# HarryShomer/LPFormer

Hardware: AMD Instinct MI355X
Metric: candidate link-pairs scored/sec (whole node) (higher is better)
Workload: dtype f32

## Files before the change

### lpformer_amd/csrc/tail_chain.hip

```cpp
#include <type_traits>

#include "lpf_common.h"

namespace {

typedef float f32x4 __attribute__((ext_vector_type(4)));

#ifndef LPF_TC_GROUPS
#define LPF_TC_GROUPS 4
#endif
constexpr int TC_GROUPS = LPF_TC_GROUPS;
constexpr int TC_WAVES = 2 * TC_GROUPS;
constexpr int TC_THREADS = 64 * TC_WAVES;

struct TailArgs {
    int64_t M;
    const float *x; int64_t ldx; int KA;
    const float *addend; int64_t ldadd;
    const float *wA, *lnA_g, *lnA_b; int NA;
    const float *tail; int64_t ldtail;
    const float *wB, *bB, *lnB_g, *lnB_b; int NB;
    const float *re; int64_t ldre;
    const float *wC, *bC; int NC;
    const float *wdot, *bdot;
    float *logit, *prob;
    const float *part;
    const float *bnd;
    int64_t units_cap;
    const int32_t *type_ptr;
    const float *att_bias;
    const int64_t *sel_ctl;
    int n_counts;
    const float *rows; int64_t ldrows;
    const int32_t *perm;
    const int64_t *n_full;
    const float *bC_empty;
    const float *row_empty;
    const float *X; int64_t ldX;
    const int64_t *batch; int64_t batch_ld, n_rows;
    const float *wE, *bE, *lnE_g, *lnE_b;
};

constexpr int tc_per_thread(int ntp) { return (ntp * 64 + TC_THREADS - 1) / TC_THREADS; }
constexpr int tc_stage_stride(int ntp) { return (ntp * 64 + 511) / 512 * 512; }

typedef short bf16x4_bits __attribute__((ext_vector_type(4)));
template <int P, int NTP, typename T>
__device__ __forceinline__ void tc_load(T (&r)[P], const float *packed, int stage, int tid) {
    const T *src = reinterpret_cast<const T *>(packed) + (int64_t)stage * tc_stage_stride(NTP);
#pragma unroll
    for (int e = 0; e < P; ++e) {
        const int i = e * TC_THREADS + tid;
#ifdef TC_NOWLOAD
        r[e] = T{};
        (void)src; (void)i;
#else
        r[e] = src[i < tc_stage_stride(NTP) ? i : 0];
#endif
    }
}
template <int P, typename T>
__device__ __forceinline__ void tc_store(const T (&r)[P], T *slab, int tid) {
#pragma unroll
    for (int e = 0; e < P; ++e) slab[e * TC_THREADS + tid] = r[e];
}

template <int TPW>
__device__ __forceinline__ void tc_mfma(f32x4 (&acc)[TPW], const f32x4 *lw, const f32x4 bv, bool last = true) {
    f32x4 a[TPW];
#pragma unroll
    for (int c = 0; c < TPW; ++c) a[c] = lw[c * 64];
#pragma unroll
    for (int u = 0; u < 4; ++u) {
#pragma unroll
        for (int c = 0; c < TPW - 1; ++c) acc[c] = __builtin_amdgcn_mfma_f32_16x16x4f32(a[c][u], bv[u], acc[c], 0, 0, 0);
        if (last) acc[TPW - 1] = __builtin_amdgcn_mfma_f32_16x16x4f32(a[TPW - 1][u], bv[u], acc[TPW - 1], 0, 0, 0);
    }
}
template <int TPW>
__device__ __forceinline__ void tc_mfma(f32x4 (&acc)[TPW], const uint2 *lw, const f32x4 bv, bool last = true) {
    bf16x4_bits b;
#pragma unroll
    for (int u = 0; u < 4; ++u) b[u] = (short)lpf_f32_to_bf16(bv[u]);
#pragma unroll
    for (int c = 0; c < TPW; ++c) {
        if (c == TPW - 1 && !last) break;
        const uint2 w = lw[c * 64];
        const bf16x4_bits a = {(short)(w.x & 0xffffu), (short)(w.x >> 16), (short)(w.y & 0xffffu), (short)(w.y >> 16)};
        acc[c] = __builtin_amdgcn_mfma_f32_16x16x16bf16_1k(a, b, acc[c], 0, 0, 0);
    }
}

template <int TPW>
__device__ __forceinline__ void tc_layernorm(f32x4 (&acc)[TPW], int fbase, int n, const float *g, const float *b, int half,
                                             int q, float *my_x, const float *peer_x, bool relu) {
    float s1 = 0.f;
#pragma unroll
    for (int c = 0; c < TPW; ++c) s1 += acc[c][0] + acc[c][1] + acc[c][2] + acc[c][3];
    s1 = lpf_quad_sum(s1);
    __syncthreads();
    if (q == 0) *my_x = s1;
    __syncthreads();
    const float mean = (half == 0 ? s1 + *peer_x : *peer_x + s1) / (float)n;
    float s2 = 0.f;
#pragma unroll
    for (int c = 0; c < TPW; ++c)
#pragma unroll
        for (int r = 0; r < 4; ++r) {
            const float d = (fbase + 16 * c + r < n) ? acc[c][r] - mean : 0.f;
            s2 += d * d;
        }
    s2 = lpf_quad_sum(s2);
    __syncthreads();
    if (q == 0) *my_x = s2;
    __syncthreads();
    const float rstd = 1.0f / sqrtf((half == 0 ? s2 + *peer_x : *peer_x + s2) / (float)n + 1e-5f);
#pragma unroll
    for (int c = 0; c < TPW; ++c) {
        const f32x4 gg = *reinterpret_cast<const f32x4 *>(g + fbase + 16 * c);
        const f32x4 bb = *reinterpret_cast<const f32x4 *>(b + fbase + 16 * c);
        acc[c] = (acc[c] - mean) * rstd * gg + bb;
        if (relu) {
#pragma unroll
            for (int r = 0; r < 4; ++r) acc[c][r] = fmaxf(acc[c][r], 0.f);
        }
    }
}

#ifdef TC_STAMPS
__device__ uint64_t *tc_stamp_buf = nullptr;
#define TC_STAMP(k) do { if (lane == 0) st_t[k] = wall_clock64(); } while (0)
#define TC_STAMPS_OUT(kind) do { if (lane == 0 && tc_stamp_buf) { uint64_t *o__ = tc_stamp_buf + ((int64_t)blockIdx.x * TC_WAVES + wave) * 16; \
        for (int k__ = 0; k__ < 8; ++k__) o__[k__] = st_t[k__]; o__[15] = (kind); } } while (0)
#else
#define TC_STAMP(k) do { } while (0)
#define TC_STAMPS_OUT(kind) do { } while (0)
#endif

template <int NTA, int NTB, int NTC>
struct TcShape {
    static constexpr int NTPA = (NTA + 1) & ~1, NTPB = (NTB + 1) & ~1, NTPC = (NTC + 1) & ~1;
    static constexpr int PA = tc_per_thread(NTPA), PB = tc_per_thread(NTPB), PC = tc_per_thread(NTPC);
    static constexpr int PM = PA > PB ? (PA > PC ? PA : PC) : (PB > PC ? PB : PC);
    static constexpr int SLAB = PM * TC_THREADS;
    static constexpr int HT = NTPA > NTPB ? NTPA : NTPB;
    static constexpr int HID = TC_GROUPS * HT * 64;
    static constexpr size_t BYTES = (size_t)(2 * SLAB + HID) * sizeof(f32x4) + TC_WAVES * 16 * sizeof(float);
};

template <int NTA, int NTB, int NTC, int WM = 0, bool ROWS = false, bool EW = false>
__global__ __launch_bounds__(TC_THREADS, NTC >= 32 ? 2 : (TC_THREADS >= 512 ? 4 : 3)) void tail_chain_kernel(const TailArgs A) {
    using S = TcShape<NTA, NTB, NTC>;
    constexpr bool WB = WM != 0;
    using WT = typename std::conditional<WM == 1, uint2, f32x4>::type;
    constexpr int NTPA = S::NTPA, NTPB = S::NTPB, NTPC = S::NTPC;
    constexpr int TPWA = NTPA / 2, TPWB = NTPB / 2, TPWC = NTPC / 2;
    constexpr int NGE = NTA;
    extern __shared__ __attribute__((aligned(16))) f32x4 lds[];
    f32x4 *hid = lds + 2 * S::SLAB;
    float *xch = reinterpret_cast<float *>(hid + S::HID);
    const int tid = threadIdx.x, lane = tid & 63, wave = tid >> 6;
    const int grp = wave >> 1, half = wave & 1, q = lane >> 4, j = lane & 15;
    float *my_x = xch + wave * 16 + j;
    const float *peer_x = xch + (wave ^ 1) * 16 + j;
    f32x4 *my_hid = hid + (grp * S::HT) * 64 + lane;
    int buf = 0;
#ifdef TC_STAMPS
    uint64_t st_t[8] = {0};
    TC_STAMP(0);
#endif

    const int64_t tile = blockIdx.x;
    const int64_t pos = tile * (16 * TC_GROUPS) + grp * 16 + j;
    const bool live = pos < A.M;
    bool lite = false;
    int64_t m = pos;
    if constexpr (ROWS) {
        if (A.perm) {
            m = A.perm[live ? pos : A.M - 1];
            lite = tile * (16 * TC_GROUPS) >= *A.n_full;
        }
    }
    const int64_t mm = live ? m : (ROWS && A.perm ? m : A.M - 1);
    bool no_sel = false;
    if constexpr (ROWS) no_sel = A.perm && A.row_empty && (live ? pos : A.M - 1) >= *A.n_full;

    f32x4 accC[TPWC];
    if constexpr (EW) {
        static_assert(ROWS && WM == 0 && S::PA == 1 && NTPA == NTA && NGE % 2 == 0 && 2 * tc_stage_stride(NTPA) <= S::SLAB &&
                          tc_stage_stride(2 * NTPA) == 2 * tc_stage_stride(NTPA), "stage E: the fp32 rows form at D = 128");
        int64_t ra = A.batch[mm], rb = A.batch[A.batch_ld + mm];
        if ((uint64_t)ra >= (uint64_t)A.n_rows) ra = 0;
        if ((uint64_t)rb >= (uint64_t)A.n_rows) rb = 0;
        const float *xa = A.X + ra * A.ldX + 4 * q, *xb = A.X + rb * A.ldX + 4 * q;
        f32x4 accE[TPWA];
#pragma unroll
        for (int c = 0; c < TPWA; ++c) accE[c] = (f32x4){0.f, 0.f, 0.f, 0.f};
        WT wrE[2];
        tc_load<2, 2 * NTPA>(wrE, A.wE, 0, tid);
        f32x4 xra[NGE], xrb[NGE];
#pragma unroll
        for (int kg = 0; kg < NGE; ++kg) {
            xra[kg] = *reinterpret_cast<const f32x4 *>(xa + 16 * kg);
            xrb[kg] = *reinterpret_cast<const f32x4 *>(xb + 16 * kg);
        }
#pragma unroll
        for (int kg = 0; kg < NGE; kg += 2) {
            const f32x4 bv0 = xra[kg] * xrb[kg], bv1 = xra[kg + 1] * xrb[kg + 1];
            WT *lw = reinterpret_cast<WT *>(lds) + buf * S::SLAB;
            tc_store<2>(wrE, lw, tid);
            __syncthreads();
            if (kg + 2 < NGE) tc_load<2, 2 * NTPA>(wrE, A.wE, kg / 2 + 1, tid);
            tc_mfma<TPWA>(accE, lw + (half * TPWA) * 64 + lane, bv0);
            tc_mfma<TPWA>(accE, lw + tc_stage_stride(NTPA) + (half * TPWA) * 64 + lane, bv1);
            buf ^= 1;
        }
        WT wrCe[S::PC];
        tc_load<S::PC, NTPC>(wrCe, A.wC, 0, tid);
        {
            const int fbase = 16 * half * TPWA + 4 * q;
#pragma unroll
            for (int c = 0; c < TPWA; ++c) accE[c] += *reinterpret_cast<const f32x4 *>(A.bE + fbase + 16 * c);
            tc_layernorm<TPWA>(accE, fbase, A.NA, A.lnE_g, A.lnE_b, half, q, my_x, peer_x, true);
#pragma unroll
            for (int c = 0; c < TPWA; ++c) my_hid[(half * TPWA + c) * 64] = accE[c];
        }
        TC_STAMP(7);
#pragma unroll
        for (int c = 0; c < TPWC; ++c) accC[c] = (f32x4){0.f, 0.f, 0.f, 0.f};
#pragma unroll 1
        for (int kg = 0; kg < NGE; ++kg) {
            WT *lw = reinterpret_cast<WT *>(lds) + buf * S::SLAB;
            tc_store<S::PC>(wrCe, lw, tid);
            __syncthreads();
            if (kg + 1 < NGE) tc_load<S::PC, NTPC>(wrCe, A.wC, kg + 1, tid);
            tc_mfma<TPWC>(accC, lw + (half * TPWC) * 64 + lane, my_hid[kg * 64]);
            buf ^= 1;
        }
        TC_STAMP(4);
        if (!lite) __syncthreads();
    }

    if constexpr (ROWS) {
        if (lite) {
            f32x4 (&acc)[TPWC] = accC;
            if constexpr (!EW) {
#pragma unroll
            for (int c = 0; c < TPWC; ++c) acc[c] = (f32x4){0.f, 0.f, 0.f, 0.f};
            WT wr[S::PC];
            const float *rer = A.re + mm * A.ldre + 4 * q;
            tc_load<S::PC, NTPC>(wr, A.wC, 0, tid);
            f32x4 xr = *reinterpret_cast<const f32x4 *>(rer);
#pragma unroll 1
            for (int kg = 0; kg < NGE; ++kg) {
                const f32x4 bv = xr;
                WT *lw = reinterpret_cast<WT *>(lds) + buf * S::SLAB;
                tc_store<S::PC>(wr, lw, tid);
                __syncthreads();
                if (kg + 1 < NGE) {
                    tc_load<S::PC, NTPC>(wr, A.wC, kg + 1, tid);
                    xr = *reinterpret_cast<const f32x4 *>(rer + 16 * (kg + 1));
                }
                tc_mfma<TPWC>(acc, lw + (half * TPWC) * 64 + lane, bv);
                buf ^= 1;
            }
            }
            const int fbase = 16 * half * TPWC + 4 * q;
            float d = 0.f;
#pragma unroll
            for (int c = 0; c < TPWC; ++c) {
                const f32x4 b = *reinterpret_cast<const f32x4 *>(A.bC_empty + fbase + 16 * c);
                const f32x4 w = *reinterpret_cast<const f32x4 *>(A.wdot + fbase + 16 * c);
#pragma unroll
                for (int r = 0; r < 4; ++r) d = fmaf(fmaxf(acc[c][r] + b[r], 0.f), w[r], d);
            }
            d = lpf_quad_sum(d);
            if (q == 0) *my_x = d;
            __syncthreads();
            if (live && q == 0 && half == 0) {
                d = d + *peer_x + A.bdot[0];
                if (A.sel_ctl && A.sel_ctl[3] != 0) d = __builtin_nanf("");
                if (A.logit) A.logit[m] = d;
                if (A.prob) A.prob[m] = 1.0f / (1.0f + expf(-d));
            }
            TC_STAMP(6);
            TC_STAMPS_OUT(1);
            return;
        }
    }
    f32x4 accA[TPWA];
#pragma unroll
    for (int c = 0; c < TPWA; ++c) accA[c] = (f32x4){0.f, 0.f, 0.f, 0.f};
    int seg_cnt[3] = {0, 0, 0};
    if (!WB && !ROWS && A.part == nullptr) {
        const float *xa = A.x + mm * A.ldx;
        const int ngA = (A.KA + 15) >> 4;
        f32x4 wr[S::PA];
        tc_load<S::PA, NTPA>(wr, A.wA, 0, tid);
        int kk = 4 * q < A.KA ? 4 * q : A.KA - 4;
        f32x4 xr = *reinterpret_cast<const f32x4 *>(xa + kk);
#pragma unroll 1
        for (int kg = 0; kg < ngA; ++kg) {
            const f32x4 bv = (16 * kg + 4 * q < A.KA) ? xr : (f32x4){0.f, 0.f, 0.f, 0.f};
            f32x4 *lw = lds + buf * S::SLAB;
            tc_store<S::PA>(wr, lw, tid);
            __syncthreads();
            if (kg + 1 < ngA) {
                tc_load<S::PA, NTPA>(wr, A.wA, kg + 1, tid);
                kk = 16 * (kg + 1) + 4 * q;
                kk = kk < A.KA ? kk : A.KA - 4;
                xr = *reinterpret_cast<const f32x4 *>(xa + kk);
            }
            tc_mfma<TPWA>(accA, lw + (half * TPWA) * 64 + lane, bv);
            buf ^= 1;
        }
    }
    WT wrB[S::PB];
    tc_load<S::PB, NTPB>(wrB, A.wB, 0, tid);
    if constexpr (ROWS) {
        const int fbase = 16 * half * TPWA + 4 * q;
        const float *row = no_sel ? A.row_empty : A.rows + mm * A.ldrows;
#pragma unroll
        for (int c = 0; c < TPWA; ++c) {
            const int f0 = fbase + 16 * c;
            const f32x4 v = *reinterpret_cast<const f32x4 *>(row + (f0 < A.NA ? f0 : 0));
            accA[c] = f0 < A.NA ? v : (f32x4){0.f, 0.f, 0.f, 0.f};
        }
    } else if (A.part == nullptr) {
        const int fbase = 16 * half * TPWA + 4 * q;
        f32x4 ad[TPWA];
#pragma unroll
        for (int c = 0; c < TPWA; ++c) {
            const int f0 = fbase + 16 * c;
            ad[c] = *reinterpret_cast<const f32x4 *>(A.addend + mm * A.ldadd + (f0 < A.NA ? f0 : 0));
        }
#pragma unroll
        for (int c = 0; c < TPWA; ++c) accA[c] += (fbase + 16 * c < A.NA) ? ad[c] : (f32x4){0.f, 0.f, 0.f, 0.f};
    } else {
        const int fbase = 16 * half * TPWA + 4 * q;
        const int64_t rs = A.NA + 4;
        float mx = -INFINITY, den = 0.f;
        f32x4 v[TPWA];
#pragma unroll
        for (int c = 0; c < TPWA; ++c) v[c] = (f32x4){0.f, 0.f, 0.f, 0.f};
        auto fetch = [&](const float *rec, f32x4 &h, f32x4 *b) __attribute__((always_inline)) {
            h = *reinterpret_cast<const f32x4 *>(rec + A.NA);
#pragma unroll
            for (int c = 0; c < TPWA; ++c) {
                const int f0 = fbase + 16 * c;
                b[c] = *reinterpret_cast<const f32x4 *>(rec + (f0 < A.NA ? f0 : 0));
            }
        };
        auto merge = [&](const f32x4 &h, const f32x4 *b) __attribute__((always_inline)) {
            const float mn = fmaxf(mx, h[0]);
            const float sa = __expf(mx - mn), sb = __expf(h[0] - mn);
            den = fmaf(den, sa, h[1] * sb);
#pragma unroll
            for (int c = 0; c < TPWA; ++c) v[c] = v[c] * sa + b[c] * sb;
            mx = mn;
        };
        int lo[3], hi[3], n_p[3];
#pragma unroll
        for (int t = 0; t < 3; ++t) {
            const int32_t *tp = A.type_ptr + (int64_t)t * (A.M + 1) + mm;
            lo[t] = tp[0];
            hi[t] = tp[1];
        }
        {
            f32x4 h0[3], b0[3][TPWA];
#pragma unroll
            for (int t = 0; t < 3; ++t) {
                seg_cnt[t] = hi[t] - lo[t];
                const bool some = hi[t] > lo[t] && ((hi[t] - 1) >> 4) < A.units_cap;
                n_p[t] = some ? ((hi[t] - 1) >> 4) - (lo[t] >> 4) + 1 : 0;
                const float *rec = n_p[t] > 1 ? A.bnd + ((((int64_t)t * A.units_cap + (lo[t] >> 4)) * 2) + 1) * rs
                                              : A.part + ((int64_t)t * A.M + mm) * rs;
                h0[t] = (f32x4){0.f, 0.f, 0.f, 0.f};
#pragma unroll
                for (int c = 0; c < TPWA; ++c) b0[t][c] = (f32x4){0.f, 0.f, 0.f, 0.f};
                if (n_p[t] > 0) fetch(rec, h0[t], b0[t]);
            }
#pragma unroll
            for (int t = 0; t < 3; ++t)
                if (n_p[t] > 0) merge(h0[t], b0[t]);
        }
        const int r0 = n_p[0] > 1 ? n_p[0] - 1 : 0, r1 = n_p[1] > 1 ? n_p[1] - 1 : 0, r2 = n_p[2] > 1 ? n_p[2] - 1 : 0;
        const int n_rest = r0 + r1 + r2;
        constexpr int NB = TPWA >= 4 ? 2 : 4;
#pragma unroll 1
        for (int k0 = 0; k0 < n_rest; k0 += NB) {
            f32x4 hh[NB], bb[NB][TPWA];
#pragma unroll
            for (int i = 0; i < NB; ++i) {
                const int k = k0 + i < n_rest ? k0 + i : n_rest - 1;
                const int t = k < r0 ? 0 : (k < r0 + r1 ? 1 : 2);
                const int jj = k - (t == 0 ? 0 : (t == 1 ? r0 : r0 + r1));
                const int ut = t == 0 ? lo[0] >> 4 : (t == 1 ? lo[1] >> 4 : lo[2] >> 4);
                fetch(A.bnd + (((int64_t)t * A.units_cap + ut + 1 + jj) * 2) * rs, hh[i], bb[i]);
            }
#pragma unroll
            for (int i = 0; i < NB; ++i)
                if (k0 + i < n_rest) merge(hh[i], bb[i]);
        }
        const float inv = 1.0f / (den + 1e-16f);
#pragma unroll
        for (int c = 0; c < TPWA; ++c) {
            const int f0 = fbase + 16 * c;
            if (f0 < A.NA) accA[c] = v[c] * inv + *reinterpret_cast<const f32x4 *>(A.att_bias + f0);
        }
    }
    {
        const int fbase = 16 * half * TPWA + 4 * q;
        if constexpr (!ROWS) tc_layernorm<TPWA>(accA, fbase, A.NA, A.lnA_g, A.lnA_b, half, q, my_x, peer_x, false);
#pragma unroll
        for (int c = 0; c < TPWA; ++c) my_hid[(half * TPWA + c) * 64] = accA[c];
    }

    TC_STAMP(1);
    f32x4 accB[TPWB];
#pragma unroll
    for (int c = 0; c < TPWB; ++c) accB[c] = (f32x4){0.f, 0.f, 0.f, 0.f};
    {
        f32x4 tailv = (f32x4){0.f, 0.f, 0.f, 0.f};
        if (q == 0) {
            if constexpr (ROWS) {
                if (!no_sel) tailv = *reinterpret_cast<const f32x4 *>(A.rows + mm * A.ldrows + A.NA);
            } else if (A.part == nullptr) {
                tailv = *reinterpret_cast<const f32x4 *>(A.tail + mm * A.ldtail);
            } else {
                const float n0 = (float)seg_cnt[0], n1 = (float)seg_cnt[1], n2 = (float)seg_cnt[2];
                tailv = A.n_counts == 4 ? (f32x4){n0, n1, n2, n0 + n1}
                                         : (A.n_counts == 3 ? (f32x4){n0, n1, n0 + n1, 0.f} : (f32x4){n0, 0.f, 0.f, 0.f});
            }
        }
#pragma unroll
        for (int kg = 0; kg < NTPA + 1; ++kg) {
            WT *lw = reinterpret_cast<WT *>(lds) + buf * S::SLAB;
            tc_store<S::PB>(wrB, lw, tid);
            __syncthreads();
            if (kg + 1 < NTPA + 1) tc_load<S::PB, NTPB>(wrB, A.wB, kg + 1, tid);
            const f32x4 bv = kg < NTPA ? my_hid[(kg < NTPA ? kg : 0) * 64] : tailv;
            tc_mfma<TPWB>(accB, lw + (half * TPWB) * 64 + lane, bv, !((NTB & 1) && half == 1));
            buf ^= 1;
        }
    }
    TC_STAMP(2);
    WT wrC[S::PC];
    tc_load<S::PC, NTPC>(wrC, A.wC, EW ? NGE : 0, tid);
    const float *rer = EW ? nullptr : A.re + mm * A.ldre + 4 * q;
    f32x4 xr = (f32x4){0.f, 0.f, 0.f, 0.f};
    if constexpr (!EW) xr = *reinterpret_cast<const f32x4 *>(rer);
    {
        const int fbase = 16 * half * TPWB + 4 * q;
#pragma unroll
        for (int c = 0; c < TPWB; ++c) accB[c] += *reinterpret_cast<const f32x4 *>(A.bB + fbase + 16 * c);
        tc_layernorm<TPWB>(accB, fbase, A.NB, A.lnB_g, A.lnB_b, half, q, my_x, peer_x, true);
#pragma unroll
        for (int c = 0; c < TPWB; ++c) my_hid[(half * TPWB + c) * 64] = accB[c];
    }

    TC_STAMP(3);
    if constexpr (!EW) {
#pragma unroll
    for (int c = 0; c < TPWC; ++c) accC[c] = (f32x4){0.f, 0.f, 0.f, 0.f};
#pragma unroll 1
    for (int kg = 0; kg < NGE; ++kg) {
        const f32x4 bv = xr;
        WT *lw = reinterpret_cast<WT *>(lds) + buf * S::SLAB;
        tc_store<S::PC>(wrC, lw, tid);
        __syncthreads();
        tc_load<S::PC, NTPC>(wrC, A.wC, kg + 1, tid);
        if (kg + 1 < NGE) xr = *reinterpret_cast<const f32x4 *>(rer + 16 * (kg + 1));
        tc_mfma<TPWC>(accC, lw + (half * TPWC) * 64 + lane, bv);
        buf ^= 1;
    }
    TC_STAMP(4);
    }
#pragma unroll
    for (int kg = 0; kg < NTB; ++kg) {
        WT *lw = reinterpret_cast<WT *>(lds) + buf * S::SLAB;
        tc_store<S::PC>(wrC, lw, tid);
        __syncthreads();
        if (kg + 1 < NTB) tc_load<S::PC, NTPC>(wrC, A.wC, NGE + kg + 1, tid);
        tc_mfma<TPWC>(accC, lw + (half * TPWC) * 64 + lane, my_hid[kg * 64]);
        buf ^= 1;
    }
    TC_STAMP(5);
    {
        const int fbase = 16 * half * TPWC + 4 * q;
        float d = 0.f;
#pragma unroll
        for (int c = 0; c < TPWC; ++c) {
            const f32x4 b = *reinterpret_cast<const f32x4 *>(A.bC + fbase + 16 * c);
            const f32x4 w = *reinterpret_cast<const f32x4 *>(A.wdot + fbase + 16 * c);
#pragma unroll
            for (int r = 0; r < 4; ++r) d = fmaf(fmaxf(accC[c][r] + b[r], 0.f), w[r], d);
        }
        d = lpf_quad_sum(d);
        __syncthreads();
        if (q == 0) *my_x = d;
        __syncthreads();
        if (live && q == 0 && half == 0) {
            d = d + *peer_x + A.bdot[0];
            if (A.sel_ctl && A.sel_ctl[3] != 0) d = __builtin_nanf("");
            if (A.logit) A.logit[m] = d;
            if (A.prob) A.prob[m] = 1.0f / (1.0f + expf(-d));
        }
    }
    TC_STAMP(6);
    TC_STAMPS_OUT(0);
}

template <int NTA, int NTB, int NTC, int WM = 0, bool ROWS = false, bool EW = false>
int tc_launch(const TailArgs &a, hipStream_t s) {
    constexpr size_t lds = TcShape<NTA, NTB, NTC>::BYTES;
    auto kern = tail_chain_kernel<NTA, NTB, NTC, WM, ROWS, EW>;
    LPF_SET_MAX_LDS(kern, lds);
    const int64_t blocks = (a.M + 16 * TC_GROUPS - 1) / (16 * TC_GROUPS);
    if (blocks > 0x7fffffff) return LPF_ERR_UNSUPPORTED;
    hipLaunchKernelGGL(kern, dim3((unsigned)blocks), dim3(TC_THREADS), lds, s, a);
    LPF_CHECK_LAUNCH();
    return LPF_OK;
}

}

#ifdef TC_STAMPS
extern "C" int lpf_tail_chain_set_stamps(void *buf) {
    return hipMemcpyToSymbol(HIP_SYMBOL(tc_stamp_buf), &buf, sizeof(buf)) == hipSuccess ? LPF_OK : LPF_ERR_LAUNCH;
}
#endif


extern "C" int lpf_tail_chain_f32(int64_t M, int32_t D, int32_t n_counts, const float *G, int64_t ldg,
                                  const float *wA_packed, const float *lnA_g, const float *lnA_b, const float *counts,
                                  int64_t ldc, const float *wB_packed, const float *bB, const float *lnB_g,
                                  const float *lnB_b, const float *r_e, int64_t ldre, const float *wC_packed,
                                  const float *bC, const float *w_dot, const float *b_dot, float *logit, float *prob,
                                  void *stream) {
    if (M == 0) return LPF_OK;
    LPF_REQUIRE(M > 0 && G && wA_packed && lnA_g && lnA_b && counts && wB_packed && bB && lnB_g && lnB_b && r_e &&
                wC_packed && bC && w_dot && b_dot && (logit || prob));
    LPF_REQUIRE(n_counts >= 1 && n_counts <= 4 && (ldg & 3) == 0 && ldg >= 4 * D + 4 && (ldc & 3) == 0 && ldc >= 4 &&
                (ldre & 3) == 0 && ldre >= D);
    LPF_REQUIRE(lpf_aligned16(G) && lpf_aligned16(counts) && lpf_aligned16(r_e) && lpf_aligned16(wA_packed) &&
                lpf_aligned16(wB_packed) && lpf_aligned16(wC_packed) && lpf_aligned16(lnA_g) && lpf_aligned16(lnA_b) &&
                lpf_aligned16(bB) && lpf_aligned16(lnB_g) && lpf_aligned16(lnB_b) && lpf_aligned16(bC) &&
                lpf_aligned16(w_dot));
    TailArgs a{M, G + D, ldg, 3 * D + 4, G, ldg, wA_packed, lnA_g, lnA_b, D, counts, ldc, wB_packed, bB, lnB_g,
               lnB_b, D + n_counts, r_e, ldre, wC_packed, bC, 2 * D, w_dot, b_dot, logit, prob,
               nullptr, nullptr, 0, nullptr, nullptr, nullptr, n_counts, nullptr, 0, nullptr, nullptr, nullptr, nullptr};
    hipStream_t s = static_cast<hipStream_t>(stream);
    switch (D) {
        case 32: return tc_launch<2, 3, 4>(a, s);
        case 64: return tc_launch<4, 5, 8>(a, s);
        case 128: return tc_launch<8, 9, 16>(a, s);
        default: return LPF_ERR_UNSUPPORTED;
    }
}

extern "C" int lpf_tail_chain_merge_f32(int64_t M, int32_t D, int32_t n_counts, const float *part, const float *bnd,
                                        int64_t units_cap, const int32_t *type_ptr, const float *att_bias, const float *lnA_g,
                                        const float *lnA_b, const float *wB_packed, const float *bB, const float *lnB_g,
                                        const float *lnB_b, const float *r_e, int64_t ldre, const float *wC_packed,
                                        const float *bC, const float *w_dot, const float *b_dot,
                                        const int64_t *sel_ctl, float *logit, float *prob, void *stream) {
    if (M == 0) return LPF_OK;
    LPF_REQUIRE(M > 0 && part && bnd && units_cap > 0 && lpf_aligned16(bnd) && type_ptr && att_bias && lnA_g && lnA_b && wB_packed && bB && lnB_g && lnB_b && r_e &&
                wC_packed && bC && w_dot && b_dot && (logit || prob));
    LPF_REQUIRE((n_counts == 1 || n_counts == 3 || n_counts == 4) && (ldre & 3) == 0 && ldre >= D);
    LPF_REQUIRE(lpf_aligned16(part) && lpf_aligned16(att_bias) && lpf_aligned16(r_e) && lpf_aligned16(wB_packed) &&
                lpf_aligned16(wC_packed) && lpf_aligned16(lnA_g) && lpf_aligned16(lnA_b) && lpf_aligned16(bB) &&
                lpf_aligned16(lnB_g) && lpf_aligned16(lnB_b) && lpf_aligned16(bC) && lpf_aligned16(w_dot));
    TailArgs a{M, nullptr, 0, 0, nullptr, 0, nullptr, lnA_g, lnA_b, D, nullptr, 0, wB_packed, bB, lnB_g,
               lnB_b, D + n_counts, r_e, ldre, wC_packed, bC, 2 * D, w_dot, b_dot, logit, prob,
               part, bnd, units_cap, type_ptr, att_bias, sel_ctl, n_counts, nullptr, 0, nullptr, nullptr, nullptr, nullptr};
    hipStream_t s = static_cast<hipStream_t>(stream);
    switch (D) {
        case 32: return tc_launch<2, 3, 4>(a, s);
        case 64: return tc_launch<4, 5, 8>(a, s);
        case 128: return tc_launch<8, 9, 16>(a, s);
        default: return LPF_ERR_UNSUPPORTED;
    }
}

extern "C" int lpf_tail_chain_merge_bf16(int64_t M, int32_t D, int32_t n_counts, const float *part, const float *bnd,
                                         int64_t units_cap, const int32_t *type_ptr, const float *att_bias,
                                         const float *lnA_g, const float *lnA_b, const void *wB_packed_bf16,
                                         const float *bB, const float *lnB_g, const float *lnB_b, const float *r_e,
                                         int64_t ldre, const void *wC_packed_bf16, const float *bC, const float *w_dot,
                                         const float *b_dot, const int64_t *sel_ctl, float *logit, float *prob,
                                         void *stream) {
    if (M == 0) return LPF_OK;
    LPF_REQUIRE(M > 0 && part && bnd && units_cap > 0 && lpf_aligned16(bnd) && type_ptr && att_bias && lnA_g && lnA_b &&
                wB_packed_bf16 && bB && lnB_g && lnB_b && r_e && wC_packed_bf16 && bC && w_dot && b_dot &&
                (logit || prob));
    LPF_REQUIRE((n_counts == 1 || n_counts == 3 || n_counts == 4) && (ldre & 3) == 0 && ldre >= D);
    LPF_REQUIRE(lpf_aligned16(part) && lpf_aligned16(att_bias) && lpf_aligned16(r_e) && lpf_aligned16(wB_packed_bf16) &&
                lpf_aligned16(wC_packed_bf16) && lpf_aligned16(lnA_g) && lpf_aligned16(lnA_b) && lpf_aligned16(bB) &&
                lpf_aligned16(lnB_g) && lpf_aligned16(lnB_b) && lpf_aligned16(bC) && lpf_aligned16(w_dot));
    TailArgs a{M, nullptr, 0, 0, nullptr, 0, nullptr, lnA_g, lnA_b, D, nullptr, 0,
               static_cast<const float *>(wB_packed_bf16), bB, lnB_g, lnB_b, D + n_counts, r_e, ldre,
               static_cast<const float *>(wC_packed_bf16), bC, 2 * D, w_dot, b_dot, logit, prob,
               part, bnd, units_cap, type_ptr, att_bias, sel_ctl, n_counts, nullptr, 0, nullptr, nullptr, nullptr, nullptr};
    hipStream_t s = static_cast<hipStream_t>(stream);
    switch (D) {
        case 32: return tc_launch<2, 3, 4, 1>(a, s);
        case 64: return tc_launch<4, 5, 8, 1>(a, s);
        case 128: return tc_launch<8, 9, 16, 1>(a, s);
        default: return LPF_ERR_UNSUPPORTED;
    }
}

namespace {
template <int WM>
int tc_rows(int64_t M, int32_t D, int32_t n_counts, const float *rows, int64_t ldrows, const void *wB, const float *bB,
            const float *lnB_g, const float *lnB_b, const float *r_e, int64_t ldre, const void *wC, const float *bC,
            const float *w_dot, const float *b_dot, const int64_t *sel_ctl, float *logit, float *prob, void *stream,
            const int32_t *perm = nullptr, const int64_t *n_full = nullptr, const float *bC_empty = nullptr,
            const float *row_empty = nullptr) {
    if (M == 0) return LPF_OK;
    LPF_REQUIRE(!perm || (n_full && bC_empty && lpf_aligned16(bC_empty)));
    LPF_REQUIRE(!row_empty || (perm && lpf_aligned16(row_empty)));
    LPF_REQUIRE(M > 0 && rows && wB && bB && lnB_g && lnB_b && r_e && wC && bC && w_dot && b_dot && (logit || prob));
    LPF_REQUIRE((n_counts == 1 || n_counts == 3 || n_counts == 4) && (ldre & 3) == 0 && ldre >= D && (ldrows & 3) == 0 &&
                ldrows >= D + 4);
    LPF_REQUIRE(lpf_aligned16(rows) && lpf_aligned16(r_e) && lpf_aligned16(wB) && lpf_aligned16(wC) && lpf_aligned16(bB) &&
                lpf_aligned16(lnB_g) && lpf_aligned16(lnB_b) && lpf_aligned16(bC) && lpf_aligned16(w_dot));
    TailArgs a{M, nullptr, 0, 0, nullptr, 0, nullptr, nullptr, nullptr, D, nullptr, 0, static_cast<const float *>(wB), bB,
               lnB_g, lnB_b, D + n_counts, r_e, ldre, static_cast<const float *>(wC), bC, 2 * D, w_dot, b_dot, logit, prob,
               nullptr, nullptr, 0, nullptr, nullptr, sel_ctl, n_counts, rows, ldrows, perm, n_full, bC_empty, row_empty};
    hipStream_t s = static_cast<hipStream_t>(stream);
    switch (D) {
        case 32: return tc_launch<2, 3, 4, WM, true>(a, s);
        case 64: return tc_launch<4, 5, 8, WM, true>(a, s);
        case 128: return tc_launch<8, 9, 16, WM, true>(a, s);
        case 256: return tc_launch<16, 17, 32, WM, true>(a, s);
        default: return LPF_ERR_UNSUPPORTED;
    }
}
}

extern "C" int lpf_tail_chain_rows_f32(int64_t M, int32_t D, int32_t n_counts, const float *rows, int64_t ldrows,
                                       const float *wB_packed, const float *bB, const float *lnB_g, const float *lnB_b,
                                       const float *r_e, int64_t ldre, const float *wC_packed, const float *bC,
                                       const float *w_dot, const float *b_dot, const int64_t *sel_ctl, float *logit,
                                       float *prob, void *stream) {
    return tc_rows<0>(M, D, n_counts, rows, ldrows, wB_packed, bB, lnB_g, lnB_b, r_e, ldre, wC_packed, bC, w_dot, b_dot,
                          sel_ctl, logit, prob, stream);
}

extern "C" int lpf_tail_chain_rows_bf16(int64_t M, int32_t D, int32_t n_counts, const float *rows, int64_t ldrows,
                                        const void *wB_packed_bf16, const float *bB, const float *lnB_g, const float *lnB_b,
                                        const float *r_e, int64_t ldre, const void *wC_packed_bf16, const float *bC,
                                        const float *w_dot, const float *b_dot, const int64_t *sel_ctl, float *logit,
                                        float *prob, void *stream) {
    return tc_rows<1>(M, D, n_counts, rows, ldrows, wB_packed_bf16, bB, lnB_g, lnB_b, r_e, ldre, wC_packed_bf16, bC, w_dot,
                         b_dot, sel_ctl, logit, prob, stream);
}

extern "C" int lpf_tail_chain_rows_perm_f32(int64_t M, int32_t D, int32_t n_counts, const float *rows, int64_t ldrows,
                                            const float *wB_packed, const float *bB, const float *lnB_g,
                                            const float *lnB_b, const float *r_e, int64_t ldre, const float *wC_packed,
                                            const float *bC, const float *w_dot, const float *b_dot,
                                            const int64_t *sel_ctl, const int32_t *perm, const int64_t *n_full,
                                            const float *bC_empty, const float *row_empty, float *logit, float *prob,
                                            void *stream) {
    LPF_REQUIRE(perm && n_full && bC_empty);
    return tc_rows<0>(M, D, n_counts, rows, ldrows, wB_packed, bB, lnB_g, lnB_b, r_e, ldre, wC_packed, bC, w_dot, b_dot,
                          sel_ctl, logit, prob, stream, perm, n_full, bC_empty, row_empty);
}

extern "C" int lpf_tail_chain_rows_perm_bf16(int64_t M, int32_t D, int32_t n_counts, const float *rows, int64_t ldrows,
                                             const void *wB_packed_bf16, const float *bB, const float *lnB_g,
                                             const float *lnB_b, const float *r_e, int64_t ldre,
                                             const void *wC_packed_bf16, const float *bC, const float *w_dot,
                                             const float *b_dot, const int64_t *sel_ctl, const int32_t *perm,
                                             const int64_t *n_full, const float *bC_empty, const float *row_empty,
                                             float *logit, float *prob, void *stream) {
    LPF_REQUIRE(perm && n_full && bC_empty);
    return tc_rows<1>(M, D, n_counts, rows, ldrows, wB_packed_bf16, bB, lnB_g, lnB_b, r_e, ldre, wC_packed_bf16, bC, w_dot,
                         b_dot, sel_ctl, logit, prob, stream, perm, n_full, bC_empty, row_empty);
}

extern "C" int lpf_tail_chain_rows_perm_ew_f32(int64_t M, int32_t D, int32_t n_counts, const float *rows, int64_t ldrows,
                                               const float *wB_packed, const float *bB, const float *lnB_g,
                                               const float *lnB_b, const float *r_e, int64_t ldre, const float *wC_packed,
                                               const float *bC, const float *w_dot, const float *b_dot,
                                               const int64_t *sel_ctl, const int32_t *perm, const int64_t *n_full,
                                               const float *bC_empty, const float *row_empty, const float *X, int64_t ldx,
                                               const int64_t *batch, int64_t batch_ld, int64_t n_rows,
                                               const float *wE_packed, const float *bE, const float *lnE_g,
                                               const float *lnE_b, float *logit, float *prob, void *stream) {
    if (!wE_packed)
        return lpf_tail_chain_rows_perm_f32(M, D, n_counts, rows, ldrows, wB_packed, bB, lnB_g, lnB_b, r_e, ldre, wC_packed, bC,
                                            w_dot, b_dot, sel_ctl, perm, n_full, bC_empty, row_empty, logit, prob, stream);
    if (M == 0) return LPF_OK;
    if (D != 128) return LPF_ERR_UNSUPPORTED;
    LPF_REQUIRE(perm && n_full && bC_empty && lpf_aligned16(bC_empty) && (!row_empty || lpf_aligned16(row_empty)));
    LPF_REQUIRE(M > 0 && rows && wB_packed && bB && lnB_g && lnB_b && wC_packed && bC && w_dot && b_dot && (logit || prob));
    LPF_REQUIRE((n_counts == 1 || n_counts == 3 || n_counts == 4) && (ldrows & 3) == 0 && ldrows >= D + 4);
    LPF_REQUIRE(X && batch && bE && lnE_g && lnE_b && n_rows > 0 && batch_ld >= M && (ldx & 3) == 0 && ldx >= D);
    LPF_REQUIRE(lpf_aligned16(rows) && lpf_aligned16(wB_packed) && lpf_aligned16(wC_packed) && lpf_aligned16(bB) &&
                lpf_aligned16(lnB_g) && lpf_aligned16(lnB_b) && lpf_aligned16(bC) && lpf_aligned16(w_dot) &&
                lpf_aligned16(X) && lpf_aligned16(wE_packed) && lpf_aligned16(bE) && lpf_aligned16(lnE_g) &&
                lpf_aligned16(lnE_b));
    TailArgs a{M, nullptr, 0, 0, nullptr, 0, nullptr, nullptr, nullptr, D, nullptr, 0, wB_packed, bB,
               lnB_g, lnB_b, D + n_counts, nullptr, 0, wC_packed, bC, 2 * D, w_dot, b_dot, logit, prob,
               nullptr, nullptr, 0, nullptr, nullptr, sel_ctl, n_counts, rows, ldrows, perm, n_full, bC_empty, row_empty,
               X, ldx, batch, batch_ld, n_rows, wE_packed, bE, lnE_g, lnE_b};
    return tc_launch<8, 9, 16, 0, true, true>(a, static_cast<hipStream_t>(stream));
}
```

Baseline: 270.5 million.

## Stage bias/LN vectors in LDS, split exchange slots, prefetch rows, pin MFMA schedule

Bias, LayerNorm gain/shift and dot-weight vectors are loaded into registers at kernel start and published to a new LDS region, so the epilogues read them from LDS rather than global memory. The cross-wave exchange buffer is widened to five slots, which lets several __syncthreads calls in the layernorm and final-dot reductions be dropped. In the stage-E path the per-row feature loads are issued early so their latency overlaps other work. Scheduling barriers are placed around the MFMA loops to fix instruction order. The cost is more LDS per block, with a static assert checking two blocks still fit per CU, plus extra registers held across the kernel, which could reduce occupancy.

New measurement: 274.1 million, median of 6. +1.3%, better.

```diff
diff --git a/lpformer_amd/csrc/tail_chain.hip b/lpformer_amd/csrc/tail_chain.hip
--- a/lpformer_amd/csrc/tail_chain.hip
+++ b/lpformer_amd/csrc/tail_chain.hip
@@ -65,6 +65,8 @@
     for (int e = 0; e < P; ++e) slab[e * TC_THREADS + tid] = r[e];
 }
 
+#define TC_PIN() __builtin_amdgcn_sched_barrier(0)
+
 template <int TPW>
 __device__ __forceinline__ void tc_mfma(f32x4 (&acc)[TPW], const f32x4 *lw, const f32x4 bv, bool last = true) {
     f32x4 a[TPW];
@@ -91,6 +93,7 @@
     }
 }
 
+constexpr int TC_XCH_SLOT = TC_WAVES * 16;
 template <int TPW>
 __device__ __forceinline__ void tc_layernorm(f32x4 (&acc)[TPW], int fbase, int n, const float *g, const float *b, int half,
                                              int q, float *my_x, const float *peer_x, bool relu) {
@@ -98,7 +101,6 @@
 #pragma unroll
     for (int c = 0; c < TPW; ++c) s1 += acc[c][0] + acc[c][1] + acc[c][2] + acc[c][3];
     s1 = lpf_quad_sum(s1);
-    __syncthreads();
     if (q == 0) *my_x = s1;
     __syncthreads();
     const float mean = (half == 0 ? s1 + *peer_x : *peer_x + s1) / (float)n;
@@ -111,10 +113,10 @@
             s2 += d * d;
         }
     s2 = lpf_quad_sum(s2);
+    if (q == 0) my_x[TC_XCH_SLOT] = s2;
     __syncthreads();
-    if (q == 0) *my_x = s2;
-    __syncthreads();
-    const float rstd = 1.0f / sqrtf((half == 0 ? s2 + *peer_x : *peer_x + s2) / (float)n + 1e-5f);
+    const float p2 = peer_x[TC_XCH_SLOT];
+    const float rstd = 1.0f / sqrtf((half == 0 ? s2 + p2 : p2 + s2) / (float)n + 1e-5f);
 #pragma unroll
     for (int c = 0; c < TPW; ++c) {
         const f32x4 gg = *reinterpret_cast<const f32x4 *>(g + fbase + 16 * c);
@@ -145,7 +147,10 @@
     static constexpr int SLAB = PM * TC_THREADS;
     static constexpr int HT = NTPA > NTPB ? NTPA : NTPB;
     static constexpr int HID = TC_GROUPS * HT * 64;
-    static constexpr size_t BYTES = (size_t)(2 * SLAB + HID) * sizeof(f32x4) + TC_WAVES * 16 * sizeof(float);
+    static constexpr int XCH = 5 * TC_WAVES * 16;
+    static constexpr int VEC_B = 3 * 16 * NTPA, VEC_C = VEC_B + 3 * 16 * NTPB, VEC_N = VEC_C + 2 * 16 * NTPC;
+    static constexpr size_t BYTES = (size_t)(2 * SLAB + HID) * sizeof(f32x4) + (XCH + VEC_N) * sizeof(float);
+    static_assert(NTC >= 32 || BYTES <= 81920, "two workgroups share a CU's 160 KB of LDS");
 };
 
 template <int NTA, int NTB, int NTC, int WM = 0, bool ROWS = false, bool EW = false>
@@ -163,6 +168,7 @@
     const int grp = wave >> 1, half = wave & 1, q = lane >> 4, j = lane & 15;
     float *my_x = xch + wave * 16 + j;
     const float *peer_x = xch + (wave ^ 1) * 16 + j;
+    float *vec = xch + S::XCH;
     f32x4 *my_hid = hid + (grp * S::HT) * 64 + lane;
     int buf = 0;
 #ifdef TC_STAMPS
@@ -185,25 +191,74 @@
     bool no_sel = false;
     if constexpr (ROWS) no_sel = A.perm && A.row_empty && (live ? pos : A.M - 1) >= *A.n_full;
 
+    constexpr int VP0 = EW ? 0 : S::VEC_B / 4, VPN = S::VEC_N / 4 - VP0, VPT = (VPN + TC_THREADS - 1) / TC_THREADS;
+    f32x4 vecr[VPT];
+#pragma unroll
+    for (int e = 0; e < VPT; ++e) {
+        int p = VP0 + e * TC_THREADS + tid;
+        p = p < S::VEC_N / 4 ? p : S::VEC_N / 4 - 1;
+        const float *src;
+        if (p >= S::VEC_C / 4) {
+            const int o = p - S::VEC_C / 4;
+            src = o < 4 * NTPC ? (lite ? A.bC_empty : A.bC) + 4 * o : A.wdot + 4 * (o - 4 * NTPC);
+        } else if (!EW || p >= S::VEC_B / 4) {
+            const int o = p - S::VEC_B / 4;
+            src = o < 4 * NTPB ? A.bB + 4 * o : (o < 8 * NTPB ? A.lnB_g + 4 * (o - 4 * NTPB) : A.lnB_b + 4 * (o - 8 * NTPB));
+        } else {
+            src = p < 4 * NTPA ? A.bE + 4 * p : (p < 8 * NTPA ? A.lnE_g + 4 * (p - 4 * NTPA) : A.lnE_b + 4 * (p - 8 * NTPA));
+        }
+        vecr[e] = *reinterpret_cast<const f32x4 *>(src);
+    }
+    TC_PIN();
+    auto tc_vec_publish = [&]() __attribute__((always_inline)) {
+#pragma unroll
+        for (int e = 0; e < VPT; ++e) {
+            int p = VP0 + e * TC_THREADS + tid;
+            p = p < S::VEC_N / 4 ? p : S::VEC_N / 4 - 1;
+            reinterpret_cast<f32x4 *>(vec)[p] = vecr[e];
+        }
+    };
+    const float *v_bE = vec, *v_lnE_g = vec + 16 * NTPA, *v_lnE_b = vec + 32 * NTPA;
+    const float *v_bB = vec + S::VEC_B, *v_lnB_g = v_bB + 16 * NTPB, *v_lnB_b = v_bB + 32 * NTPB;
+    const float *v_bC = vec + S::VEC_C, *v_wdot = v_bC + 16 * NTPC;
+
+    f32x4 rowv[ROWS ? TPWA : 1], rowt = (f32x4){0.f, 0.f, 0.f, 0.f};
+#pragma unroll
+    for (int c = 0; c < (ROWS ? TPWA : 1); ++c) rowv[c] = (f32x4){0.f, 0.f, 0.f, 0.f};
+    auto tc_rows_request = [&]() __attribute__((always_inline)) {
+        if constexpr (ROWS) {
+            const int fbase = 16 * half * TPWA + 4 * q;
+            const float *own = A.rows + mm * A.ldrows, *row = no_sel ? A.row_empty : own;
+#pragma unroll
+            for (int c = 0; c < TPWA; ++c) {
+                const int f0 = fbase + 16 * c;
+                rowv[c] = *reinterpret_cast<const f32x4 *>(row + (f0 < A.NA ? f0 : 0));
+            }
+            rowt = *reinterpret_cast<const f32x4 *>(own + A.NA);
+        }
+    };
+
     f32x4 accC[TPWC];
     if constexpr (EW) {
         static_assert(ROWS && WM == 0 && S::PA == 1 && NTPA == NTA && NGE % 2 == 0 && 2 * tc_stage_stride(NTPA) <= S::SLAB &&
                           tc_stage_stride(2 * NTPA) == 2 * tc_stage_stride(NTPA), "stage E: the fp32 rows form at D = 128");
         int64_t ra = A.batch[mm], rb = A.batch[A.batch_ld + mm];
+        WT wrE[2];
+        tc_load<2, 2 * NTPA>(wrE, A.wE, 0, tid);
+        TC_PIN();
         if ((uint64_t)ra >= (uint64_t)A.n_rows) ra = 0;
         if ((uint64_t)rb >= (uint64_t)A.n_rows) rb = 0;
         const float *xa = A.X + ra * A.ldX + 4 * q, *xb = A.X + rb * A.ldX + 4 * q;
         f32x4 accE[TPWA];
 #pragma unroll
         for (int c = 0; c < TPWA; ++c) accE[c] = (f32x4){0.f, 0.f, 0.f, 0.f};
-        WT wrE[2];
-        tc_load<2, 2 * NTPA>(wrE, A.wE, 0, tid);
         f32x4 xra[NGE], xrb[NGE];
 #pragma unroll
         for (int kg = 0; kg < NGE; ++kg) {
             xra[kg] = *reinterpret_cast<const f32x4 *>(xa + 16 * kg);
             xrb[kg] = *reinterpret_cast<const f32x4 *>(xb + 16 * kg);
         }
+        tc_vec_publish();
 #pragma unroll
         for (int kg = 0; kg < NGE; kg += 2) {
             const f32x4 bv0 = xra[kg] * xrb[kg], bv1 = xra[kg + 1] * xrb[kg + 1];
@@ -211,17 +266,20 @@
             tc_store<2>(wrE, lw, tid);
             __syncthreads();
             if (kg + 2 < NGE) tc_load<2, 2 * NTPA>(wrE, A.wE, kg / 2 + 1, tid);
+            TC_PIN();
             tc_mfma<TPWA>(accE, lw + (half * TPWA) * 64 + lane, bv0);
             tc_mfma<TPWA>(accE, lw + tc_stage_stride(NTPA) + (half * TPWA) * 64 + lane, bv1);
+            TC_PIN();
             buf ^= 1;
         }
+        if (!lite) tc_rows_request();
         WT wrCe[S::PC];
         tc_load<S::PC, NTPC>(wrCe, A.wC, 0, tid);
         {
             const int fbase = 16 * half * TPWA + 4 * q;
 #pragma unroll
-            for (int c = 0; c < TPWA; ++c) accE[c] += *reinterpret_cast<const f32x4 *>(A.bE + fbase + 16 * c);
-            tc_layernorm<TPWA>(accE, fbase, A.NA, A.lnE_g, A.lnE_b, half, q, my_x, peer_x, true);
+            for (int c = 0; c < TPWA; ++c) accE[c] += *reinterpret_cast<const f32x4 *>(v_bE + fbase + 16 * c);
+            tc_layernorm<TPWA>(accE, fbase, A.NA, v_lnE_g, v_lnE_b, half, q, my_x, peer_x, true);
 #pragma unroll
             for (int c = 0; c < TPWA; ++c) my_hid[(half * TPWA + c) * 64] = accE[c];
         }
@@ -251,6 +309,7 @@
             const float *rer = A.re + mm * A.ldre + 4 * q;
             tc_load<S::PC, NTPC>(wr, A.wC, 0, tid);
             f32x4 xr = *reinterpret_cast<const f32x4 *>(rer);
+            tc_vec_publish();
 #pragma unroll 1
             for (int kg = 0; kg < NGE; ++kg) {
                 const f32x4 bv = xr;
@@ -269,16 +328,16 @@
             float d = 0.f;
 #pragma unroll
             for (int c = 0; c < TPWC; ++c) {
-                const f32x4 b = *reinterpret_cast<const f32x4 *>(A.bC_empty + fbase + 16 * c);
-                const f32x4 w = *reinterpret_cast<const f32x4 *>(A.wdot + fbase + 16 * c);
+                const f32x4 b = *reinterpret_cast<const f32x4 *>(v_bC + fbase + 16 * c);
+                const f32x4 w = *reinterpret_cast<const f32x4 *>(v_wdot + fbase + 16 * c);
 #pragma unroll
                 for (int r = 0; r < 4; ++r) d = fmaf(fmaxf(acc[c][r] + b[r], 0.f), w[r], d);
             }
             d = lpf_quad_sum(d);
-            if (q == 0) *my_x = d;
+            if (q == 0) my_x[4 * TC_XCH_SLOT] = d;
             __syncthreads();
             if (live && q == 0 && half == 0) {
-                d = d + *peer_x + A.bdot[0];
+                d = d + peer_x[4 * TC_XCH_SLOT] + A.bdot[0];
                 if (A.sel_ctl && A.sel_ctl[3] != 0) d = __builtin_nanf("");
                 if (A.logit) A.logit[m] = d;
                 if (A.prob) A.prob[m] = 1.0f / (1.0f + expf(-d));
@@ -288,6 +347,7 @@
             return;
         }
     }
+    if constexpr (!EW) tc_vec_publish();
     f32x4 accA[TPWA];
 #pragma unroll
     for (int c = 0; c < TPWA; ++c) accA[c] = (f32x4){0.f, 0.f, 0.f, 0.f};
@@ -319,13 +379,9 @@
     tc_load<S::PB, NTPB>(wrB, A.wB, 0, tid);
     if constexpr (ROWS) {
         const int fbase = 16 * half * TPWA + 4 * q;
-        const float *row = no_sel ? A.row_empty : A.rows + mm * A.ldrows;
-#pragma unroll
-        for (int c = 0; c < TPWA; ++c) {
-            const int f0 = fbase + 16 * c;
-            const f32x4 v = *reinterpret_cast<const f32x4 *>(row + (f0 < A.NA ? f0 : 0));
-            accA[c] = f0 < A.NA ? v : (f32x4){0.f, 0.f, 0.f, 0.f};
-        }
+        if constexpr (!EW) tc_rows_request();
+#pragma unroll
+        for (int c = 0; c < TPWA; ++c) accA[c] = fbase + 16 * c < A.NA ? rowv[c] : (f32x4){0.f, 0.f, 0.f, 0.f};
     } else if (A.part == nullptr) {
         const int fbase = 16 * half * TPWA + 4 * q;
         f32x4 ad[TPWA];
@@ -422,10 +478,10 @@
     for (int c = 0; c < TPWB; ++c) accB[c] = (f32x4){0.f, 0.f, 0.f, 0.f};
     {
         f32x4 tailv = (f32x4){0.f, 0.f, 0.f, 0.f};
-        if (q == 0) {
-            if constexpr (ROWS) {
-                if (!no_sel) tailv = *reinterpret_cast<const f32x4 *>(A.rows + mm * A.ldrows + A.NA);
-            } else if (A.part == nullptr) {
+        if constexpr (ROWS) {
+            if (q == 0 && !no_sel) tailv = rowt;
+        } else if (q == 0) {
+            if (A.part == nullptr) {
                 tailv = *reinterpret_cast<const f32x4 *>(A.tail + mm * A.ldtail);
             } else {
                 const float n0 = (float)seg_cnt[0], n1 = (float)seg_cnt[1], n2 = (float)seg_cnt[2];
@@ -453,8 +509,8 @@
     {
         const int fbase = 16 * half * TPWB + 4 * q;
 #pragma unroll
-        for (int c = 0; c < TPWB; ++c) accB[c] += *reinterpret_cast<const f32x4 *>(A.bB + fbase + 16 * c);
-        tc_layernorm<TPWB>(accB, fbase, A.NB, A.lnB_g, A.lnB_b, half, q, my_x, peer_x, true);
+        for (int c = 0; c < TPWB; ++c) accB[c] += *reinterpret_cast<const f32x4 *>(v_bB + fbase + 16 * c);
+        tc_layernorm<TPWB>(accB, fbase, A.NB, v_lnB_g, v_lnB_b, half, q, my_x + 2 * TC_XCH_SLOT, peer_x + 2 * TC_XCH_SLOT, true);
 #pragma unroll
         for (int c = 0; c < TPWB; ++c) my_hid[(half * TPWB + c) * 64] = accB[c];
     }
@@ -482,7 +538,9 @@
         tc_store<S::PC>(wrC, lw, tid);
         __syncthreads();
         if (kg + 1 < NTB) tc_load<S::PC, NTPC>(wrC, A.wC, NGE + kg + 1, tid);
+        TC_PIN();
         tc_mfma<TPWC>(accC, lw + (half * TPWC) * 64 + lane, my_hid[kg * 64]);
+        TC_PIN();
         buf ^= 1;
     }
     TC_STAMP(5);
@@ -491,17 +549,16 @@
         float d = 0.f;
 #pragma unroll
         for (int c = 0; c < TPWC; ++c) {
-            const f32x4 b = *reinterpret_cast<const f32x4 *>(A.bC + fbase + 16 * c);
-            const f32x4 w = *reinterpret_cast<const f32x4 *>(A.wdot + fbase + 16 * c);
+            const f32x4 b = *reinterpret_cast<const f32x4 *>(v_bC + fbase + 16 * c);
+            const f32x4 w = *reinterpret_cast<const f32x4 *>(v_wdot + fbase + 16 * c);
 #pragma unroll
             for (int r = 0; r < 4; ++r) d = fmaf(fmaxf(accC[c][r] + b[r], 0.f), w[r], d);
         }
         d = lpf_quad_sum(d);
-        __syncthreads();
-        if (q == 0) *my_x = d;
+        if (q == 0) my_x[4 * TC_XCH_SLOT] = d;
         __syncthreads();
         if (live && q == 0 && half == 0) {
-            d = d + *peer_x + A.bdot[0];
+            d = d + peer_x[4 * TC_XCH_SLOT] + A.bdot[0];
             if (A.sel_ctl && A.sel_ctl[3] != 0) d = __builtin_nanf("");
             if (A.logit) A.logit[m] = d;
             if (A.prob) A.prob[m] = 1.0f / (1.0f + expf(-d));
```
